# mmetcalf14/qml-cutensornet

Measured on AMD Instinct MI355X. Metric: Gram kernel entries/sec @ 60 qubits x 6 layers, higher is better.
Workload: dtype f64 (complex128)

## Files before the change

### __graft_entry__.py

```python
from __future__ import annotations

import os
import shutil
import subprocess
import sys

ROOT = os.path.dirname(os.path.abspath(__file__))
PKG = os.path.join(ROOT, "qml-cutensornet_amd")
if ROOT not in sys.path:
    sys.path.insert(0, ROOT)


def _run(cmd):
    print("+", " ".join(cmd), file=sys.stderr, flush=True)
    subprocess.run(cmd, check=True)


def _stale(out, deps):
    return not os.path.exists(out) or os.path.getmtime(out) < max(os.path.getmtime(f) for f in deps)


def build_variant(name, defines) -> str:
    build()
    hipcc = shutil.which("hipcc") or "/opt/rocm/bin/hipcc"
    csrc, lab = os.path.join(PKG, "csrc"), os.path.join(ROOT, "lab")
    obj, out = os.path.join(lab, f"qkgram_{name}.o"), os.path.join(lab, f"libqkgram_{name}.so")
    srcs = [os.path.join(csrc, f) for f in ("qkgram.hip", "qk_fused.h", "qk_ring.h", "qk_device.h", "qk_host.h", "qk_devmem.h", "qk_plan.h")] + [os.path.join(lab, "qk_quad.h")]
    if _stale(out, srcs):
        _run([hipcc, "--offload-arch=gfx950", "-O3", "-std=c++17", "-fPIC", "-DQKF_EXPERIMENT", "-I", lab] + [f"-D{d}" for d in defines] + ["-c", "-o", obj, srcs[0]])
        _run([hipcc, "--offload-arch=gfx950", "-shared", "-fPIC", "-o", out, obj] + [os.path.join(csrc, f) for f in ("qk_build.o", "qk_comm.o", "qk_local.o", "qk_planner.o")] + ["-ldl", "-lpthread"])
    return out


def build() -> None:
    hipcc = shutil.which("hipcc") or "/opt/rocm/bin/hipcc"
    csrc = os.path.join(PKG, "csrc")
    lab = os.path.join(ROOT, "lab")
    inc = os.path.join(ROOT, "include", "qkgram.h")
    common = [os.path.join(csrc, h) for h in ("qk_host.h", "qk_devmem.h", "qk_plan.h", "qk_device.h")] + [inc]
    deps = {
        "qkgram.hip": common + [os.path.join(csrc, h) for h in ("qk_ring.h", "qk_fused.h")],
        "qk_build.hip": common + [os.path.join(csrc, "qk_build_kernels.h")],
        "qk_comm.hip": common,
        "qk_local.hip": common + [os.path.join(csrc, "qk_ring.h")],
    }
    gxx = shutil.which("g++") or "g++"
    psrc, pobj = os.path.join(csrc, "qk_planner.cpp"), os.path.join(csrc, "qk_planner.o")
    if _stale(pobj, [psrc, os.path.join(csrc, "qk_plan.h"), inc]):
        _run([gxx, "-O3", "-std=c++17", "-fPIC", "-pthread", "-fopenmp-simd", "-c", "-o", pobj, psrc])
    targets = [(os.path.join(PKG, "libqkgram.so"), "", [], [])]
    if os.path.exists(os.path.join(lab, "qk_lab.hip")):
        targets.append((os.path.join(lab, "libqklab.so"), ".lab", ["-DQK_LAB", "-I", csrc, "-I", lab], [os.path.join(lab, "qk_lab.hip")]))
    for out, tag, flags, extra in targets:
        objs = []
        for src in [os.path.join(csrc, f) for f in deps] + extra:
            obj = os.path.splitext(src)[0] + tag + ".o"
            d = deps.get(os.path.basename(src), deps["qkgram.hip"] + [os.path.join(lab, "qk_lab.h")])
            if _stale(obj, [src] + d):
                _run([hipcc, "--offload-arch=gfx950", "-O3", "-std=c++17", "-fPIC"] + flags + ["-c", "-o", obj, src])
            objs.append(obj)
        if _stale(out, objs + [pobj]):
            _run([hipcc, "--offload-arch=gfx950", "-shared", "-fPIC", "-o", out] + objs + [pobj, "-ldl", "-lpthread"])
    bsrc = os.path.join(csrc, "qk_builder.cpp")
    bout = os.path.join(PKG, "libqkbuilder.so")
    if not os.path.exists(bout) or os.path.getmtime(bout) < os.path.getmtime(bsrc):
        _run([shutil.which("g++") or "g++", "-O3", "-std=c++17", "-shared", "-fPIC", "-o", bout, bsrc, "-ldl"])
    omk = os.path.join(ROOT, "oracle", "Makefile")
    if os.path.exists(omk):
        _run(["make", "-s", "-C", os.path.join(ROOT, "oracle")])
    import qml_cutensornet_amd
    from qml_cutensornet_amd import engine

    engine.lib()


def smoke() -> None:
    import numpy as np

    build()
    import qml_cutensornet_amd as Q
    from qml_cutensornet_amd import engine
    from oracle import restatement as R

    with engine.context(0) as ctx:
        ctx.selftest()
        for n, reps, gamma, d, npts, want in ((10, 2, 1.0, 2, 6, "wave"), (14, 4, 1.0, 3, 5, "fused")):
# ... 20 lines not shown
```

### lab/qk_quad.h

```cpp
#pragma once

__device__ __forceinline__ int qkq_qinv(const int d) {
  static constexpr int T[17] = {0, 1048576, 524288, 349526, 262144, 209716, 174763, 149797, 131072, 116509, 104858, 95326, 87382, 80660, 74899, 69906, 65536};
  return T[d];
}

struct QkqUnit {
  bool mine, a1, b1;
  int ta, tb, p;
};

template <bool A1, bool B1, typename XPtr>
__device__ __forceinline__ void qkq_p1(QkfTile (&T)[2][2], v2d (&fr)[4], v2d (&fs)[4], const bool primed, QkfStream cur, XPtr xp, unsigned x0, unsigned x1, const int nks,
                                       const QkfStream n0, const unsigned n1off) {
  v4d P[2][2][3];
  v2d fx[4], fy[4];
  if (!primed) qkf_load4(fr, cur);
  if (B1) {
#pragma unroll
    for (int i = 0; i < 4; ++i) fs[i] = qkf_ldg(cur.base + i * cur.step, cur.off + TILE);
  }
#pragma unroll
  for (int i = 0; i < 4; ++i) {
    fx[i] = qkf_ldx(xp + i * QKF_XSTEP, x0);
// ... 224 lines not shown
    if (cut) {
      if (un.b1) un.tb += sub, un.b1 = false;
      else if (un.a1) un.ta += sub, un.a1 = false;
      else un.mine = un.mine && sub == 0;
    }
    return un;
  };
  auto b_stream = [&](const QkfSite& s, const int s0, const QkqUnit& un) __attribute__((always_inline)) {
    return QkfStream{s.Bk + un.p * s.b2, (unsigned)((q * s.pd) * s.b2 + (s0 + un.tb) * TILE + j), 4 * s.pd * s.b2};
  };
  auto a_stream = [&](const QkfSite& s, const QkqUnit& un) __attribute__((always_inline)) {
    return QkfStream{s.Ak + un.p * s.a2, (unsigned)(((un.ta * TILE + q) * s.pd) * s.a2 + j), 4 * s.pd * s.a2};
  };
  const int xcc = qk_xcc_id();
  if (tid == 0) qk_tail_start(g);
  for (;;) {
    if (tid == 0) *slot = qk_pull(g, xcc);
    __syncthreads();
    const long long p = *slot;
    __syncthreads();
    if (p < 0) break;
    const int xi = g.pairs[2 * p], yj = g.pairs[2 * p + 1];
    qkf_step_table<XCAP, NT>(g, xi, yj, rec, m_off, tid, [](const int pmt, const int nt) { return pmt * ((nt + 1) / 2) <= NW; });
    const int ek = g.edge_k, k_hi = ns - ek;
    const bool edges = ek > 0;
    if (!edges)
      for (int e = tid; e < TILE * TILE; e += NT) XL[e] = (v2d){e == 0 ? 1.0 : 0.0, 0.0};
    __syncthreads();
    bool xg = false;
    int cur = 0, xb = 0;
    if (edges) {
      const v4i r0 = rec[3 * ek];
      const int a_e = rfl(r0.x), b_e = rfl(r0.z);
      if (a_e * b_e <= XCAP) qkf_edge_prefix<NW>(g, xi, yj, a_e, b_e, XL, wave, q, j);
      else qkf_edge_prefix<NW>(g, xi, yj, a_e, b_e, G0, wave, q, j), xg = true;
      __syncthreads();
    }
    v2d fr[4], fs[4];
    bool primed = false;
    QkfSite sn = site(ek);
    for (int k = ek; k < k_hi;) {
      const QkfSite sc = sn;
      k = sc.next;
      if (k < k_hi) sn = site(k);
      const int a = sc.a, a2 = sc.a2, b = sc.b, nt = sc.nt, W = sc.W;
      const bool small = sc.small;
      v2d* const Gc = G0 + (long long)cur * g.x_plane;
      v2d* const Gn = G0 + (long long)(cur ^ 1) * g.x_plane;
      if (small && xg) {
        for (int e = tid; e < a * b; e += NT) XL[e] = Gc[e];
        __syncthreads();
        xg = false, xb = 0;
      } else if (!small && !xg) {
        for (int e = tid; e < a * b; e += NT) Gc[e] = XL[xb + e];
        __syncthreads();
        xg = true;
      }
      const int n_out = sc.b2 * a2;
      const bool pingpong = small && a * b + n_out <= XCAP;
      const int ob = !small ? 0 : pingpong ? (xb == 0 ? XCAP - n_out : 0) : 0;
      if (pingpong)
        for (int e = tid; e < n_out; e += NT) XL[ob + e] = (v2d){0.0, 0.0};
      for (int s0 = 0; s0 < nt; s0 += W) {
        const int w = min(W, nt - s0);
        const Pieces pc = pieces_of(sc, w);
        const int quads = pc.L;
        if (!small) {
          for (int e = tid; e < w * TILE * a2; e += NT) XL[e] = (v2d){0.0, 0.0};
// ... 49 lines not shown
              constexpr bool A1_ = decltype(a1_)::value, B1_ = decltype(b1_)::value;
              if (kmax == 4) qkq_p2<true, A1_, B1_>(T, fr, fs, as, a1off, ps, sc.nn, 4, xo, q, j, nxt);
              else qkq_p2<false, A1_, B1_>(T, fr, fs, as, a1off, ps, sc.nn, kmax, xo, q, j, nxt);
            };
            if (un.a1) {
              if (un.b1) p2(std::true_type{}, std::true_type{});
              else p2(std::true_type{}, std::false_type{});
            } else {
              if (un.b1) p2(std::false_type{}, std::true_type{});
              else p2(std::false_type{}, std::false_type{});
            }
            primed = np1;
          } else {
            between();
          }
        }
        qk_lds_barrier();
        if (!small && nt > W) {
          for (int tn = 0; tn < sc.nn; ++tn)
            for (int e = tid; e < w * QKF_XBLOCK; e += NT) Gn[(long long)tn * (sc.b2 * TILE) + s0 * QKF_XBLOCK + e] = XL[tn * w * QKF_XBLOCK + e];
          __syncthreads();
        }
      }
      if (!small) {
        if (nt > W) cur ^= 1;
        else xg = false, xb = 0;
      } else {
        xb = ob;
      }
    }
    if (edges) {
      const v4i r0 = rec[3 * (k_hi - 1)];
      const int a_e = rfl(r0.y), b_e = rfl(r0.w);
      if (xg) qkf_edge_suffix<NW>(g, xi, yj, a_e, b_e, (const v2d*)(G0 + (long long)cur * g.x_plane), zacc, wave, q, j);
      else qkf_edge_suffix<NW>(g, xi, yj, a_e, b_e, (const lds_v2d*)(XL + xb), zacc, wave, q, j);
      __syncthreads();
    }
    if (tid == 0) {
      v2d zz = {0.0, 0.0};
      if (edges)
        for (int w_ = 0; w_ < NW; ++w_) zz.x += zacc[2 * w_], zz.y += zacc[2 * w_ + 1];
      else zz = xg ? G0[(long long)cur * g.x_plane] : (v2d)XL[xb];
      g.values[p] = zz.x * zz.x + zz.y * zz.y;
      if (g.z) {
        g.z[2 * p] = zz.x;
        g.z[2 * p + 1] = zz.y;
      }
    }
    __syncthreads();
  }
  if (tid == 0) qk_tail_exit(g);
}
```

### qml-cutensornet_amd/csrc/qk_fused.h

```cpp
#pragma once
#include "qk_device.h"
#include "qk_plan.h"

#define QKF_PRIO_LO() __builtin_amdgcn_s_setprio(0)
#define QKF_PRIO_HI() __builtin_amdgcn_s_setprio(2)
typedef double v2d __attribute__((ext_vector_type(2)));
typedef __attribute__((address_space(3))) v2d lds_v2d;
static constexpr int QKF_XSTEP = 4 * TILE;
static constexpr int QKF_XBLOCK = TILE * TILE;


#ifndef QKF_LDS3M
#define QKF_LDS3M 0
#endif
#ifndef QKF_P2_PROBE
#define QKF_P2_PROBE 0
#endif
#ifndef QKF_ABL
#define QKF_ABL 0
#endif
#define QKF_STEP_BARRIER()                            \
  do {                                                \
    if (QKF_ABL & 4) asm volatile("s_waitcnt lgkmcnt(0)" ::: "memory"); \
    else qk_lds_barrier();                            \
// ... 189 lines not shown
      for (int r = 0; r < 4; ++r) {
        __hip_atomic_fetch_add(d + r * 2 * QKF_XSTEP, re[r], __ATOMIC_RELAXED, __HIP_MEMORY_SCOPE_WORKGROUP);
        __hip_atomic_fetch_add(d + r * 2 * QKF_XSTEP + 1, im[r], __ATOMIC_RELAXED, __HIP_MEMORY_SCOPE_WORKGROUP);
      }
    }
    d += 2 * ps;
  }
}

template <int S>
__device__ __forceinline__ void qkf_rotate(QkfTile (&T)[S], const int L) {
  if constexpr (S >= 2) {
    if (L == 2) {
      const QkfTile t = T[S - 2];
      T[S - 2] = T[S - 1], T[S - 1] = t;
    }
  }
  if constexpr (S >= 3) {
    if (L == 3) {
      const QkfTile t = T[S - 3];
      T[S - 3] = T[S - 2], T[S - 2] = T[S - 1], T[S - 1] = t;
    }
  }
  if constexpr (S >= 4) {
    if (L >= 4) {
      const QkfTile t0 = T[0];
#pragma unroll
      for (int e = 0; e + 1 < S; ++e) T[e] = T[e + 1];
      T[S - 1] = t0;
    }
  }
}

__device__ __forceinline__ void qkf_edge_tile(QkfTile& t, const v2d* __restrict__ Ay, const int ldy, const v2d* __restrict__ Ax, const int ldx, const int ks4) {
  v4d p1 = {0, 0, 0, 0}, p2 = {0, 0, 0, 0}, p3 = {0, 0, 0, 0};
  v2d fy[4], fx[4];
#pragma unroll
  for (int i = 0; i < 4; ++i) fy[i] = Ay[(long)(4 * i) * ldy], fx[i] = Ax[(long)(4 * i) * ldx];
  for (int s0 = 0; s0 < ks4; s0 += 4) {
    const bool more = s0 + 4 < ks4;
#pragma unroll
    for (int i = 0; i < 4; ++i) {
      qkf_kstep<true>(p1, p2, p3, fy[i].x, fy[i].y, fx[i].x, fx[i].y);
      if (more) fy[i] = Ay[(long)(4 * (s0 + 4 + i)) * ldy], fx[i] = Ax[(long)(4 * (s0 + 4 + i)) * ldx];
    }
  }
  t.re = p1 + p2, t.im = p3 - p1 + p2;
}

template <int NW, typename XOut>
__device__ __forceinline__ void qkf_edge_prefix(const SweepArgs& g, const int xi, const int yj, const int a, const int b, XOut xo, const int wave, const int q, const int j) {
  const v2d* const Lx = reinterpret_cast<const v2d*>(g.xedge) + g.xedge_offs[2 * (long long)xi];
  const v2d* const Ly = reinterpret_cast<const v2d*>(g.yedge) + g.yedge_offs[2 * (long long)yj];
  const int mt = a / TILE, nt = b / TILE, ks4 = (1 << g.edge_k) >> 2;
  for (int t = wave; t < mt * nt; t += NW) {
    const int tb = t / mt, ta = t - tb * mt;
    QkfTile T;
    qkf_edge_tile(T, Ly + (long)q * b + tb * TILE + j, b, Lx + (long)q * a + ta * TILE + j, a, ks4);
#pragma unroll
    for (int r = 0; r < 4; ++r) xo[ta * (b * TILE) + (tb * TILE + q + 4 * r) * TILE + j] = (v2d){T.re[r], T.im[r]};
  }
}

template <int NW, typename XIn>
__device__ __forceinline__ void qkf_edge_suffix(const SweepArgs& g, const int xi, const int yj, const int a, const int b, XIn xin, __attribute__((address_space(3))) double* zacc, const int wave,
                                                const int q, const int j) {
  const v2d* const Rx = reinterpret_cast<const v2d*>(g.xedge) + g.xedge_offs[2 * (long long)xi + 1];
  const v2d* const Ry = reinterpret_cast<const v2d*>(g.yedge) + g.yedge_offs[2 * (long long)yj + 1];
  const int mt = a / TILE, nt = b / TILE, ks4 = (1 << g.edge_k) >> 2;
  double zr = 0, zi = 0;
  for (int t = wave; t < mt * nt; t += NW) {
    const int tb = t / mt, ta = t - tb * mt;
    QkfTile T;
    qkf_edge_tile(T, Ry + (long)q * b + tb * TILE + j, b, Rx + (long)q * a + ta * TILE + j, a, ks4);
#pragma unroll
    for (int r = 0; r < 4; ++r) {
      const v2d x = xin[ta * (b * TILE) + (tb * TILE + q + 4 * r) * TILE + j];
      zr += x.x * T.re[r] - x.y * T.im[r], zi += x.x * T.im[r] + x.y * T.re[r];
    }
  }
#pragma unroll
  for (int o = 32; o > 0; o >>= 1) zr += __shfl_xor(zr, o), zi += __shfl_xor(zi, o);
  if ((q | j) == 0) zacc[2 * wave] = zr, zacc[2 * wave + 1] = zi;
}

struct QkfSite {
  int a, a2, b, b2, at, nks, mt, nt, nn, W, inv, inv2, pd, ps, next;
  bool small;
  const v2d *Ak, *Bk;
};
typedef int v4i __attribute__((ext_vector_type(4)));
typedef __attribute__((address_space(3))) v4i lds_v4i;

template <int XCAP, int NT, bool ITEM_RECIPS = false, typename OneRound>
__device__ __forceinline__ void qkf_step_table(const SweepArgs& g, const int xi, const int yj, lds_v4i* const rec, long long* const m_off, const int tid, const OneRound one_round) {
  const int ns = g.n_sites, n1 = ns + 1;
  const int32_t* const xd = g.xdims + (long long)xi * n1;
  const int32_t* const yd = g.ydims + (long long)yj * n1;
  const int32_t* const xt = g.xtrue + (long long)xi * n1;
  const int32_t* const yt = g.ytrue + (long long)yj * n1;
  const v2d* const xdata = reinterpret_cast<const v2d*>(g.xdata);
  const v2d* const ydata = reinterpret_cast<const v2d*>(g.ydata);
  auto is_small = [&](const int a, const int a2, const int b, const int b2, const int pd) __attribute__((always_inline)) {
    return a * b <= XCAP && a2 * b2 <= XCAP && (one_round(pd * (a / TILE), b2 / TILE) || a * b + a2 * b2 <= XCAP);
  };
  auto put = [&](const int e, const int a, const int a2, const int b, const int b2, const int ps, const int next, const bool small, const v2d* const A, const v2d* const B)
                 __attribute__((always_inline)) {
    const int mt = a / TILE, nt = b2 / TILE;
    const int W = small ? nt : max(1, min(nt, XCAP / (TILE * a2)));
    rec[3 * e] = (v4i){a, a2, b, b2};
    rec[3 * e + 1] = (v4i){xt[e], (yt[e] + 3) >> 2, W, small ? 1 : 0};
// ... 20 lines not shown
    const bool sm = is_small(a, a2, b, b2, 4);
    const long long work_m = 4ll * a * b2 * (b + a2), work_p = 2ll * a * bm * (b + am) + 2ll * am * b2 * (bm + a2);
    const bool merged = (sm || (!is_small(a, am, b, bm, 2) && !is_small(am, a2, bm, b2, 2))) && work_m <= work_p;
    plain(e + 1, e + 2);
    if (merged)
      put(e, a, a2, b, b2, 2, e + 2, sm, reinterpret_cast<const v2d*>(g.xmg) + (g.xmg_offs[(long long)xi * g.merge_steps + t] >> 1),
          reinterpret_cast<const v2d*>(g.ymg) + (g.ymg_offs[(long long)yj * g.merge_steps + t] >> 1));
    else plain(e, e + 1);
  }
}

#ifdef QKF_PROF
#define QKF_PROF_DECL() \
  unsigned long long pf[8] = {0, 0, 0, 0, 0, 0, 0, 0}, pt = __builtin_amdgcn_s_memtime(); \
  const unsigned long long pt0 = pt
#define QKF_STAMP(i)                                              \
  do {                                                            \
    const unsigned long long now_ = __builtin_amdgcn_s_memtime(); \
    pf[i] += now_ - pt;                                           \
    pt = now_;                                                    \
  } while (0)
#define QKF_PROF_FLUSH()                                             \
  do {                                                               \
    if (lane == 0) {                                                 \
      pf[7] = __builtin_amdgcn_s_memtime() - pt0;                    \
      for (int i_ = 0; i_ < 8; ++i_) atomicAdd(g.prof + i_, pf[i_]); \
    }                                                                \
  } while (0)
#else
#define QKF_PROF_DECL()
#define QKF_STAMP(i)
#define QKF_PROF_FLUSH()
#endif

template <int NW, int S, int XCAP, int WPS, bool DET = false>
__global__ __launch_bounds__(64 * NW, WPS) void qk_sweep_fused_kernel(const SweepArgs g) {
  constexpr int NT = 64 * NW;
  extern __shared__ __attribute__((aligned(16))) double lds_raw[];
  lds_v2d* const XL = (lds_v2d*)lds_raw;
  long long* const slot = reinterpret_cast<long long*>(lds_raw + 2 * XCAP);
  const v2d* const xdata = reinterpret_cast<const v2d*>(g.xdata);
  const v2d* const ydata = reinterpret_cast<const v2d*>(g.ydata);
  v2d* const G0 = reinterpret_cast<v2d*>(g.scratch) + (long long)blockIdx.x * 2 * g.x_plane;
  const int tid = threadIdx.x, lane = tid & 63;
  const int wave = __builtin_amdgcn_readfirstlane(tid >> 6);
  const int j = lane & 15, q = lane >> 4;
  const int ns = g.n_sites;
  __attribute__((address_space(3))) double* const zacc = (__attribute__((address_space(3))) double*)(slot + 2);
  lds_v4i* const rec = (lds_v4i*)(slot + 2 + 32);
  long long* const m_off = reinterpret_cast<long long*>(slot + 2 + 32) + 6 * (long long)ns;
  lds_int* const tbroken = (lds_int*)(m_off + 2 * (long long)ns);
  lds_int* const turn0 = tbroken + 2;
  auto rfl = [&](const int v) __attribute__((always_inline)) { return __builtin_amdgcn_readfirstlane(v); };
  auto ldl = [&](const long long* p_) __attribute__((always_inline)) {
    const long long v = *p_;
    const unsigned lo = __builtin_amdgcn_readfirstlane((unsigned)v);
    const unsigned hi = __builtin_amdgcn_readfirstlane((unsigned)((unsigned long long)v >> 32));
    return (long long)(((unsigned long long)hi << 32) | lo);
  };
  auto site = [&](const int k) __attribute__((always_inline)) {
    const v4i r0 = rec[3 * k], r1 = rec[3 * k + 1], r2 = rec[3 * k + 2];
    QkfSite s;
    s.a = rfl(r0.x), s.a2 = rfl(r0.y), s.b = rfl(r0.z), s.b2 = rfl(r0.w);
    s.at = rfl(r1.x), s.nks = rfl(r1.y), s.W = rfl(r1.z), s.small = rfl(r1.w) != 0;
    s.inv = rfl(r2.x), s.inv2 = rfl(r2.w);
    s.ps = rfl(r2.y), s.pd = 1 << s.ps, s.next = rfl(r2.z);
// ... 12 lines not shown
  auto a_stream = [&](const QkfSite& s, const int w, const int it) __attribute__((always_inline)) {
    const QkUnit un = item_of(s, w, it);
    return QkfStream{s.Ak + un.p * s.a2, (unsigned)(((un.ta * TILE + q) * s.pd) * s.a2 + j), 4 * s.pd * s.a2, min(4, (s.at - un.ta * TILE + 3) >> 2)};
  };
  QKF_PROF_DECL();
  const int xcc = qk_xcc_id();
  int gang_round = 0;
  if (tid == 0) qk_tail_start(g);
  for (;;) {
    if (tid == 0) {
      const long long pp_ = qk_pull(g, xcc);
      qk_gang_sync(g, xcc, pp_ >= 0, gang_round);
      *slot = pp_;
    }
    __syncthreads();
    const long long p = *slot;
    __syncthreads();
    if (p < 0) break;
    const int xi = g.pairs[2 * p], yj = g.pairs[2 * p + 1];
    qkf_step_table<XCAP, NT, true>(g, xi, yj, rec, m_off, tid, [](const int pmt, const int nt) { return pmt * nt <= NW * S; });
    const int ek = g.edge_k, k_hi = ns - ek;
    const bool edges = ek > 0;
    if (!edges)
      for (int e = tid; e < TILE * TILE; e += NT) XL[e] = (v2d){e == 0 ? 1.0 : 0.0, 0.0};
    if constexpr (DET)
      for (int e = tid; e < 2 * g.turn_ints + 2; e += NT) tbroken[e] = 0;
    int tsel = 0;
    __syncthreads();
    bool xg = false;
    int cur = 0, xb = 0;
    if (edges) {
      const v4i r0 = rec[3 * ek];
      const int a_e = rfl(r0.x), b_e = rfl(r0.z);
      if (a_e * b_e <= XCAP) qkf_edge_prefix<NW>(g, xi, yj, a_e, b_e, XL, wave, q, j);
      else qkf_edge_prefix<NW>(g, xi, yj, a_e, b_e, G0, wave, q, j), xg = true;
      __syncthreads();
    }
    QKF_STAMP(0);
    QkfTile T[S];
    v2d fr[4];
    bool primed = false;
    QkfSite sn = site(ek);
    for (int k = ek; k < k_hi;) {
      const QkfSite sc = sn;
      k = sc.next;
      if (k < k_hi) sn = site(k);
      const int a = sc.a, a2 = sc.a2, b = sc.b, mt = sc.mt, nt = sc.nt, W = sc.W;
      const bool small = sc.small;
      v2d* const Gc = G0 + (long long)cur * g.x_plane;
      v2d* const Gn = G0 + (long long)(cur ^ 1) * g.x_plane;
      if (small && xg) {
        for (int e = tid; e < a * b; e += NT) XL[e] = Gc[e];
        __syncthreads();
        xg = false, xb = 0;
      } else if (!small && !xg) {
        for (int e = tid; e < a * b; e += NT) Gc[e] = XL[xb + e];
        __syncthreads();
        xg = true;
      }
      const int n_out = sc.b2 * a2;
      const bool pingpong = small && a * b + n_out <= XCAP;
      const int ob = !small ? 0 : pingpong ? (xb == 0 ? XCAP - n_out : 0) : 0;
      if (pingpong && !DET)
        for (int e = tid; e < n_out; e += NT) XL[ob + e] = (v2d){0.0, 0.0};
      QKF_STAMP(1);
      for (int s0 = 0; s0 < nt; s0 += W) {
        const int w = min(W, nt - s0), items = sc.pd * mt * w;
        lds_int* const tcur = turn0 + tsel * g.turn_ints;
// ... 44 lines not shown
            const int kmax = min(4, (sc.at - ta * TILE + 3) >> 2);
            const bool more = s + 1 < S && it + NW < items;
            const int wn = min(sn.W, sn.nt);
            const bool chain = !more && last_round && k < k_hi && wave < sn.pd * sn.mt * wn;
            const QkfStream nxt = more ? a_stream(sc, w, it + NW) : chain ? b_stream(sn, 0, wn, wave) : a_stream(sc, w, it);
            const int tix = sc.pd * ta + un.p;
            const QkfTurn turn{tcur + tbl * sc.nn, tix, tbroken, g.err};
            if (kmax == 4) qkf_p2_item<true, DET>(T[S - 1], fr, primed, a_stream(sc, w, it), w * QKF_XBLOCK, sc.nn, 4, XL + ob + tbl * QKF_XBLOCK, q, j, nxt, turn);
            else qkf_p2_item<false, DET>(T[S - 1], fr, primed, a_stream(sc, w, it), w * QKF_XBLOCK, sc.nn, kmax, XL + ob + tbl * QKF_XBLOCK, q, j, nxt, turn);
            primed = more || chain;
          }
          QKF_STAMP(4);
        }
        QKF_STEP_BARRIER();
        tsel ^= 1;
        QKF_STAMP(5);
        if (!small && nt > W) {
          for (int tn = 0; tn < sc.nn; ++tn)
            for (int e = tid; e < w * QKF_XBLOCK; e += NT) Gn[(long long)tn * (sc.b2 * TILE) + s0 * QKF_XBLOCK + e] = XL[tn * w * QKF_XBLOCK + e];
          __syncthreads();
          QKF_STAMP(1);
        }
      }
      if (!small) {
        if (nt > W) cur ^= 1;
        else xg = false, xb = 0;
      } else {
        xb = ob;
      }
    }
    if (edges) {
      const v4i r0 = rec[3 * (k_hi - 1)];
      const int a_e = rfl(r0.y), b_e = rfl(r0.w);
      if (xg) qkf_edge_suffix<NW>(g, xi, yj, a_e, b_e, (const v2d*)(G0 + (long long)cur * g.x_plane), zacc, wave, q, j);
      else qkf_edge_suffix<NW>(g, xi, yj, a_e, b_e, (const lds_v2d*)(XL + xb), zacc, wave, q, j);
      __syncthreads();
    }
    if (tid == 0) {
      v2d zz = {0.0, 0.0};
      if (edges)
        for (int w_ = 0; w_ < NW; ++w_) zz.x += zacc[2 * w_], zz.y += zacc[2 * w_ + 1];
      else zz = xg ? G0[(long long)cur * g.x_plane] : (v2d)XL[xb];
      g.values[p] = zz.x * zz.x + zz.y * zz.y;
      if (g.z) {
        g.z[2 * p] = zz.x;
        g.z[2 * p + 1] = zz.y;
      }
    }
    __syncthreads();
  }
  if (tid == 0) qk_tail_exit(g);
  QKF_PROF_FLUSH();
}

template <bool HAS1, typename XPtr>
__device__ __forceinline__ void qkf_p1_dual(QkfTile& t0, QkfTile& t1, v2d (&fr)[4], v2d (&fs)[4], const bool primed, QkfStream cur, XPtr xp, unsigned xoff, const int nks,
                                            const QkfStream nxt) {
  v4d p1 = {0, 0, 0, 0}, p2 = {0, 0, 0, 0}, p3 = {0, 0, 0, 0}, r1 = {0, 0, 0, 0}, r2 = {0, 0, 0, 0}, r3 = {0, 0, 0, 0};
  v2d fx[4];
  if (!primed) qkf_load4(fr, cur);
  if (HAS1) {
#pragma unroll
    for (int i = 0; i < 4; ++i) fs[i] = qkf_ldg(cur.base + i * cur.step, cur.off + TILE);
  }
#pragma unroll
  for (int i = 0; i < 4; ++i) fx[i] = qkf_ldx(xp + i * QKF_XSTEP, xoff);
  const int ng = (nks + 3) >> 2, last = nks - 4 * (ng - 1);
  QKF_PRIO_LO();
// ... 245 lines not shown
    s.Ak = xdata + ldl(m_off + 2 * k);
    s.Bk = ydata + ldl(m_off + 2 * k + 1);
    return s;
  };
  auto pair_of = [&](const QkfSite& s, const int v) __attribute__((always_inline)) { return qk_unit_decode_ordered(v, s.ps, s.mt, s.inv); };
  auto b_stream = [&](const QkfSite& s, const int s0, const int v, const int half) __attribute__((always_inline)) {
    const QkUnit un = pair_of(s, v);
    return QkfStream{s.Bk + un.p * s.b2, (unsigned)((q * s.pd) * s.b2 + (s0 + 2 * un.tc + half) * TILE + j), 4 * s.pd * s.b2};
  };
  struct Unit {
    bool mine, has1;
    int v, half;
  };
  auto unit_of = [&](const QkfSite& s, const int w, const int units, const int r0) __attribute__((always_inline)) {
    Unit un;
    const int left = units - r0;
    const bool halves = 2 * left <= NW;
    un.half = (halves && wave >= left) ? 1 : 0;
    un.v = r0 + wave - (un.half ? left : 0);
    const int tp = pair_of(s, un.v).tc;
    const bool second = 2 * tp + 1 < w;
    un.mine = un.v < units && (un.half == 0 || second);
    un.has1 = !halves && second;
    return un;
  };
  auto a_stream = [&](const QkfSite& s, const int v) __attribute__((always_inline)) {
    const QkUnit un = pair_of(s, v);
    return QkfStream{s.Ak + un.p * s.a2, (unsigned)(((un.ta * TILE + q) * s.pd) * s.a2 + j), 4 * s.pd * s.a2};
  };
  QKF_PROF_DECL();
  const int xcc = qk_xcc_id();
  int gang_round = 0;
  if (tid == 0) qk_tail_start(g);
  for (;;) {
    if (tid == 0) {
      const long long pp_ = qk_pull(g, xcc);
      qk_gang_sync(g, xcc, pp_ >= 0, gang_round);
      *slot = pp_;
    }
    __syncthreads();
    const long long p = *slot;
    __syncthreads();
    if (p < 0) break;
    const int xi = g.pairs[2 * p], yj = g.pairs[2 * p + 1];
    qkf_step_table<XCAP, NT>(g, xi, yj, rec, m_off, tid, [](const int pmt, const int nt) { return pmt * ((nt + 1) / 2) <= NW; });
    const int ek = g.edge_k, k_hi = ns - ek;
    const bool edges = ek > 0;
    if (!edges)
      for (int e = tid; e < TILE * TILE; e += NT) XL[e] = (v2d){e == 0 ? 1.0 : 0.0, 0.0};
    if constexpr (DET)
      for (int e = tid; e < 2 * g.turn_ints + 2; e += NT) tbroken[e] = 0;
    int tsel = 0;
    __syncthreads();
    bool xg = false;
    int cur = 0, xb = 0;
    if (edges) {
      const v4i r0 = rec[3 * ek];
      const int a_e = rfl(r0.x), b_e = rfl(r0.z);
      if (a_e * b_e <= XCAP) qkf_edge_prefix<NW>(g, xi, yj, a_e, b_e, XL, wave, q, j);
      else qkf_edge_prefix<NW>(g, xi, yj, a_e, b_e, G0, wave, q, j), xg = true;
      __syncthreads();
    }
    QKF_STAMP(0);
    QkfTile T0, T1;
    v2d fr[4], fs[4];
    bool primed = false;
    QkfSite sn = site(ek);
    for (int k = ek; k < k_hi;) {
      const QkfSite sc = sn;
      k = sc.next;
      if (k < k_hi) sn = site(k);
      const int a = sc.a, a2 = sc.a2, b = sc.b, mt = sc.mt, nt = sc.nt, W = sc.W;
      const bool small = sc.small;
      v2d* const Gc = G0 + (long long)cur * g.x_plane;
      v2d* const Gn = G0 + (long long)(cur ^ 1) * g.x_plane;
      if (small && xg) {
        for (int e = tid; e < a * b; e += NT) XL[e] = Gc[e];
        __syncthreads();
        xg = false, xb = 0;
      } else if (!small && !xg) {
        for (int e = tid; e < a * b; e += NT) Gc[e] = XL[xb + e];
        __syncthreads();
        xg = true;
      }
      const int n_out = sc.b2 * a2;
      const bool pingpong = small && a * b + n_out <= XCAP;
      const int ob = !small ? 0 : pingpong ? (xb == 0 ? XCAP - n_out : 0) : 0;
      if (pingpong && !DET)
        for (int e = tid; e < n_out; e += NT) XL[ob + e] = (v2d){0.0, 0.0};
      QKF_STAMP(1);
      for (int s0 = 0; s0 < nt; s0 += W) {
        const int w = min(W, nt - s0), units = sc.pd * mt * ((w + 1) >> 1);
        lds_int* const tcur = turn0 + tsel * g.turn_ints;
// ... 45 lines not shown
              const Unit nu = unit_of(sn, w2, sn.pd * sn.mt * ((w2 + 1) >> 1), 0);
              if (nu.mine) nxt = b_stream(sn, 0, nu.v, nu.half), np1 = true;
            }
            const unsigned nd1 = 0;
            lds_v2d* const xo = XL + ob + (2 * tp + un.half) * QKF_XBLOCK;
            const QkfTurn tp_turn{tcur + (2 * tp + un.half) * sc.nn, sc.pd * ta + pr.p, tbroken, g.err};
            if (has1) {
              if (kmax == 4) qkf_p2_dual<true, true, DET>(T0, T1, fr, fs, a_stream(sc, v), w * QKF_XBLOCK, sc.nn, 4, xo, q, j, nxt, np1, nd1, tp_turn);
              else qkf_p2_dual<false, true, DET>(T0, T1, fr, fs, a_stream(sc, v), w * QKF_XBLOCK, sc.nn, kmax, xo, q, j, nxt, np1, nd1, tp_turn);
            } else {
              if (kmax == 4) qkf_p2_dual<true, false, DET>(T0, T1, fr, fs, a_stream(sc, v), w * QKF_XBLOCK, sc.nn, 4, xo, q, j, nxt, np1, nd1, tp_turn);
              else qkf_p2_dual<false, false, DET>(T0, T1, fr, fs, a_stream(sc, v), w * QKF_XBLOCK, sc.nn, kmax, xo, q, j, nxt, np1, nd1, tp_turn);
            }
            primed = np1;
          }
          QKF_STAMP(4);
        }
        QKF_STEP_BARRIER();
        tsel ^= 1;
        QKF_STAMP(5);
        if (!small && nt > W) {
          for (int tn = 0; tn < sc.nn; ++tn)
            for (int e = tid; e < w * QKF_XBLOCK; e += NT) Gn[(long long)tn * (sc.b2 * TILE) + s0 * QKF_XBLOCK + e] = XL[tn * w * QKF_XBLOCK + e];
          __syncthreads();
        }
      }
      if (!small) {
        if (nt > W) cur ^= 1;
        else xg = false, xb = 0;
      } else {
        xb = ob;
      }
    }
    if (edges) {
      const v4i r0 = rec[3 * (k_hi - 1)];
      const int a_e = rfl(r0.y), b_e = rfl(r0.w);
      if (xg) qkf_edge_suffix<NW>(g, xi, yj, a_e, b_e, (const v2d*)(G0 + (long long)cur * g.x_plane), zacc, wave, q, j);
      else qkf_edge_suffix<NW>(g, xi, yj, a_e, b_e, (const lds_v2d*)(XL + xb), zacc, wave, q, j);
      __syncthreads();
    }
    if (tid == 0) {
      v2d zz = {0.0, 0.0};
      if (edges)
        for (int w_ = 0; w_ < NW; ++w_) zz.x += zacc[2 * w_], zz.y += zacc[2 * w_ + 1];
      else zz = xg ? G0[(long long)cur * g.x_plane] : (v2d)XL[xb];
      g.values[p] = zz.x * zz.x + zz.y * zz.y;
      if (g.z) {
        g.z[2 * p] = zz.x;
        g.z[2 * p + 1] = zz.y;
      }
    }
    __syncthreads();
    QKF_STAMP(6);
  }
  if (tid == 0) qk_tail_exit(g);
  QKF_PROF_FLUSH();
}

template <typename T>
__global__ void qk_interleave_kernel(const T* __restrict__ src, T* __restrict__ dst, const int32_t* __restrict__ dims, const int64_t* __restrict__ offs,
                                     const int n_sites, const long long n_tensors) {
  typedef T v2 __attribute__((ext_vector_type(2)));
  for (long long t = blockIdx.x; t < n_tensors; t += gridDim.x) {
    const long long s = t / n_sites;
    const int k = (int)(t - s * n_sites);
    const long long plane = (long long)dims[s * (n_sites + 1) + k] * 2 * dims[s * (n_sites + 1) + k + 1];
    const T* re = src + offs[t];
    const T* im = re + plane;
    v2* d = reinterpret_cast<v2*>(dst + offs[t]);
    for (long long e = threadIdx.x; e < plane; e += blockDim.x) d[e] = (v2){re[e], im[e]};
  }
}

template <int N>
__device__ __forceinline__ void qkw_wait_vmcnt() {
  static_assert(N >= 0 && N < 64, "vmcnt is a 6-bit field");
  asm volatile("s_waitcnt vmcnt(%0)" ::"n"(N) : "memory");
}

template <int NG, typename SRC>
__global__ __launch_bounds__(64, 2) void qk_sweep_wave2_kernel(const SweepArgs g) {
  constexpr bool F32 = sizeof(SRC) == 4;
  static_assert(!F32 || NG > 0, "complex64 images go through the LDS ring");
  constexpr int ES = F32 ? 8 : 16;
  constexpr int GROUP = F32 ? 128 : 256;
// ... 195 lines not shown
```

### qml-cutensornet_amd/csrc/qk_plan.h

```cpp
#pragma once
#include "../../include/qkgram.h"

#include <algorithm>
#include <cstdint>
#include <cstdio>
#include <vector>

int qk_fail(int code, const char* fmt, ...) __attribute__((format(printf, 2, 3)));

#ifndef QKF_XCAP_ONE_V
#define QKF_XCAP_ONE_V 8192
#endif
#ifndef QKF_XCAP_TWO_V
#define QKF_XCAP_TWO_V 4608
#endif
#ifndef QKF_TWO_WGS
#define QKF_TWO_WGS 2
#endif
static constexpr int QKF_XCAP_ONE = QKF_XCAP_ONE_V, QKF_XCAP_TWO = QKF_XCAP_TWO_V;
static constexpr int QK_TILE = 16;
static inline int qk_pad16(int x) { return (x + QK_TILE - 1) / QK_TILE * QK_TILE; }
static constexpr int GMAX = 4;

#if defined(__HIPCC__)
#define QK_HD __host__ __device__
#else
#define QK_HD
#endif
struct QkUnit {
  int ta, tc, p;
};
QK_HD static inline int qk_unit_cols(const int w, const bool dual) { return dual ? (w + 1) >> 1 : w; }
QK_HD static inline int qk_recip20(const int d) { return ((1 << 20) + d - 1) / d; }
QK_HD static inline int qk_recip15(const int d) { return ((1 << 15) + d - 1) / d; }
QK_HD static inline int qk_unit_recips(const int nt, const int W, const bool dual) {
  const int wl = nt - (nt - 1) / W * W;
  return qk_recip15(qk_unit_cols(W, dual)) | (qk_recip15(qk_unit_cols(wl, dual)) << 16);
}
QK_HD static inline int qk_unit_recip_of(const int recips, const bool full_strip) { return full_strip ? (recips & 0xffff) : (int)((unsigned)recips >> 16); }
QK_HD static inline QkUnit qk_unit_decode(const int v, const int mt, const int wc, const int inv_mt, const int inv_wc) {
  const int c = (v * inv_mt) >> 20, p = (c * inv_wc) >> 15;
  return QkUnit{v - c * mt, c - p * wc, p};
}
QK_HD static inline QkUnit qk_unit_decode_ordered(const int v, const int ps, const int mt, const int inv_mt) {
  const int u = v >> ps, tc = (u * inv_mt) >> 20;
  return QkUnit{u - tc * mt, tc, v & ((1 << ps) - 1)};
}

struct qk_ctx;

struct qk_plan {
  int n_sites = 0, nx = 0, ny = 0;
  bool symmetric = false;
  bool quad = false;
  int world = 1, rank = 0;
  int64_t total_pairs = 0, max_per_rank = 0;
  std::vector<int32_t> pairs;
  std::vector<int32_t> groups;
  int group = 1;
  qk_stats stats{};
  qk_stats second{};
  int64_t n_first = 0;
  int nq = 1;
  int64_t qstart[17] = {0};
  int edge_k = 0;
  bool second_wave2 = false;
  double fit_two = 1.0;
  double fit_narrow = 1.0;
  double tile_reuse_bytes = 0;
  double plan_ms = 0;
  int plan_threads = 1;
  qk_ctx* up_ctx = nullptr;
  int32_t* d_pairs = nullptr;
  int32_t* d_groups = nullptr;
};

struct QkSweepPolicy {
  int variant = 20;
  int wgs_per_cu = 2;
// ... 114 lines not shown
```

Measured before the change: 712,000.

## Rewrite edge prefix/suffix with pipelined MFMA groups and prefetch next pair

Replaces the edge tile contraction with a unit-based version that keeps one or two groups of k-step loads in flight, uses byte-offset addressing and scalarised base offsets, and can optionally compute two column tiles per unit. In the gang fused kernel, a dedicated puller thread fetches the next work pair during the suffix phase and the step table for the next pair is built before looping, which removes a barrier per pair. The aim is to hide global-load latency in the edge contractions and the scheduler round-trip. It adds register pressure and more complex control flow, and it changes the synchronisation ordering.

```diff
diff --git a/__graft_entry__.py b/__graft_entry__.py
--- a/__graft_entry__.py
+++ b/__graft_entry__.py
@@ -52,6 +52,9 @@
     if os.path.exists(os.path.join(lab, "qk_lab.hip")):
         targets.append((os.path.join(lab, "libqklab.so"), ".lab", ["-DQK_LAB", "-I", csrc, "-I", lab], [os.path.join(lab, "qk_lab.hip")]))
     for out, tag, flags, extra in targets:
+        every = {f for src in deps for f in [os.path.join(csrc, src)] + deps[src]} | set(extra) | {psrc, os.path.join(lab, "qk_lab.h"), os.path.join(lab, "qk_quad.h")}
+        if not _stale(out, [f for f in every if os.path.exists(f)]):
+            continue
         objs = []
         for src in [os.path.join(csrc, f) for f in deps] + extra:
             obj = os.path.splitext(src)[0] + tag + ".o"
diff --git a/lab/qk_quad.h b/lab/qk_quad.h
--- a/lab/qk_quad.h
+++ b/lab/qk_quad.h
@@ -280,8 +280,8 @@
     if (edges) {
       const v4i r0 = rec[3 * ek];
       const int a_e = rfl(r0.x), b_e = rfl(r0.z);
-      if (a_e * b_e <= XCAP) qkf_edge_prefix<NW>(g, xi, yj, a_e, b_e, XL, wave, q, j);
-      else qkf_edge_prefix<NW>(g, xi, yj, a_e, b_e, G0, wave, q, j), xg = true;
+      xg = a_e * b_e > XCAP;
+      qkf_edge_prefix<NW, QKF_EDGE_PAIRS(WPS), QKF_EDGE_SETS(WPS)>(g, xi, yj, a_e, b_e, XL, G0, xg, wave, q, j);
       __syncthreads();
     }
     v2d fr[4], fs[4];
@@ -397,8 +397,7 @@
     if (edges) {
       const v4i r0 = rec[3 * (k_hi - 1)];
       const int a_e = rfl(r0.y), b_e = rfl(r0.w);
-      if (xg) qkf_edge_suffix<NW>(g, xi, yj, a_e, b_e, (const v2d*)(G0 + (long long)cur * g.x_plane), zacc, wave, q, j);
-      else qkf_edge_suffix<NW>(g, xi, yj, a_e, b_e, (const lds_v2d*)(XL + xb), zacc, wave, q, j);
+      qkf_edge_suffix<NW, QKF_EDGE_PAIRS(WPS), QKF_EDGE_SETS(WPS)>(g, xi, yj, a_e, b_e, (const lds_v2d*)(XL + xb), (const v2d*)(G0 + (long long)cur * g.x_plane), xg, zacc, wave, q, j);
       __syncthreads();
     }
     if (tid == 0) {
diff --git a/qml-cutensornet_amd/csrc/qk_fused.h b/qml-cutensornet_amd/csrc/qk_fused.h
--- a/qml-cutensornet_amd/csrc/qk_fused.h
+++ b/qml-cutensornet_amd/csrc/qk_fused.h
@@ -245,51 +245,151 @@
   }
 }
 
-__device__ __forceinline__ void qkf_edge_tile(QkfTile& t, const v2d* __restrict__ Ay, const int ldy, const v2d* __restrict__ Ax, const int ldx, const int ks4) {
-  v4d p1 = {0, 0, 0, 0}, p2 = {0, 0, 0, 0}, p3 = {0, 0, 0, 0};
-  v2d fy[4], fx[4];
-#pragma unroll
-  for (int i = 0; i < 4; ++i) fy[i] = Ay[(long)(4 * i) * ldy], fx[i] = Ax[(long)(4 * i) * ldx];
-  for (int s0 = 0; s0 < ks4; s0 += 4) {
-    const bool more = s0 + 4 < ks4;
-#pragma unroll
-    for (int i = 0; i < 4; ++i) {
-      qkf_kstep<true>(p1, p2, p3, fy[i].x, fy[i].y, fx[i].x, fx[i].y);
-      if (more) fy[i] = Ay[(long)(4 * (s0 + 4 + i)) * ldy], fx[i] = Ax[(long)(4 * (s0 + 4 + i)) * ldx];
-    }
-  }
-  t.re = p1 + p2, t.im = p3 - p1 + p2;
-}
-
-template <int NW, typename XOut>
-__device__ __forceinline__ void qkf_edge_prefix(const SweepArgs& g, const int xi, const int yj, const int a, const int b, XOut xo, const int wave, const int q, const int j) {
-  const v2d* const Lx = reinterpret_cast<const v2d*>(g.xedge) + g.xedge_offs[2 * (long long)xi];
-  const v2d* const Ly = reinterpret_cast<const v2d*>(g.yedge) + g.yedge_offs[2 * (long long)yj];
-  const int mt = a / TILE, nt = b / TILE, ks4 = (1 << g.edge_k) >> 2;
-  for (int t = wave; t < mt * nt; t += NW) {
-    const int tb = t / mt, ta = t - tb * mt;
-    QkfTile T;
-    qkf_edge_tile(T, Ly + (long)q * b + tb * TILE + j, b, Lx + (long)q * a + ta * TILE + j, a, ks4);
-#pragma unroll
-    for (int r = 0; r < 4; ++r) xo[ta * (b * TILE) + (tb * TILE + q + 4 * r) * TILE + j] = (v2d){T.re[r], T.im[r]};
-  }
-}
-
-template <int NW, typename XIn>
-__device__ __forceinline__ void qkf_edge_suffix(const SweepArgs& g, const int xi, const int yj, const int a, const int b, XIn xin, __attribute__((address_space(3))) double* zacc, const int wave,
+#ifdef QKF_EDGE_PAIRS_V
+#define QKF_EDGE_PAIRS(WPS) (QKF_EDGE_PAIRS_V != 0)
+#else
+#define QKF_EDGE_PAIRS(WPS) false
+#endif
+#ifdef QKF_EDGE_SETS_V
+#define QKF_EDGE_SETS(WPS) (QKF_EDGE_SETS_V)
+#else
+#define QKF_EDGE_SETS(WPS) ((WPS) <= 3 ? 2 : 1)
+#endif
+__device__ __forceinline__ v2d qkf_lde(const v2d* __restrict__ base, const unsigned boff, const int col = 0) {
+  return reinterpret_cast<const v2d*>(reinterpret_cast<const char*>(base) + (size_t)boff)[col];
+}
+template <bool HAS1, bool MORE>
+__device__ __forceinline__ void qkf_edge_group(v4d (&acc)[6], v2d (&fy)[4], v2d (&fz)[4], v2d (&fx)[4], const v2d* const* const by, const v2d* const* const bx, const unsigned boy,
+                                               const unsigned box) {
+#pragma unroll
+  for (int i = 0; i < 4; ++i) {
+    const double sb = QKF_DIF(fx[i].x, fx[i].y);
+    acc[0] = __builtin_amdgcn_mfma_f64_16x16x4f64(fy[i].x, fx[i].x, acc[0], 0, 0, 0);
+    acc[1] = __builtin_amdgcn_mfma_f64_16x16x4f64(fy[i].y, fx[i].y, acc[1], 0, 0, 0);
+    acc[2] = __builtin_amdgcn_mfma_f64_16x16x4f64(QKF_SUM(fy[i].x, fy[i].y), sb, acc[2], 0, 0, 0);
+    if (HAS1) {
+      acc[3] = __builtin_amdgcn_mfma_f64_16x16x4f64(fz[i].x, fx[i].x, acc[3], 0, 0, 0);
+      acc[4] = __builtin_amdgcn_mfma_f64_16x16x4f64(fz[i].y, fx[i].y, acc[4], 0, 0, 0);
+      acc[5] = __builtin_amdgcn_mfma_f64_16x16x4f64(QKF_SUM(fz[i].x, fz[i].y), sb, acc[5], 0, 0, 0);
+    }
+    if (MORE) {
+      fy[i] = qkf_lde(by[i], boy);
+      if (HAS1) fz[i] = qkf_lde(by[i], boy, TILE);
+      fx[i] = qkf_lde(bx[i], box);
+    }
+    __builtin_amdgcn_sched_barrier(0);
+  }
+}
+template <bool HAS1, int SETS>
+__device__ __forceinline__ void qkf_edge_unit(QkfTile& t0, QkfTile& t1, const v2d* __restrict__ Ay, const unsigned oy, const int ldy, const v2d* __restrict__ Ax, const unsigned ox, const int ldx,
+                                              const int ng) {
+  static_assert(SETS == 1 || SETS == 2, "one or two groups of k-steps in flight");
+  v4d acc[6];
+#pragma unroll
+  for (int e = 0; e < 6; ++e) acc[e] = (v4d){0, 0, 0, 0};
+  v2d fy[SETS][4], fz[SETS][4], fx[SETS][4];
+  const v2d *by[4 * SETS], *bx[4 * SETS];
+#pragma unroll
+  for (int i = 0; i < 4 * SETS; ++i) by[i] = Ay + 4 * i * ldy, bx[i] = Ax + 4 * i * ldx;
+  unsigned boy = oy * 16u, box = ox * 16u;
+  const unsigned sy = (unsigned)(SETS * TILE * ldy) * 16u, sx = (unsigned)(SETS * TILE * ldx) * 16u;
+  const bool two = SETS == 2 && ng > 1;
+#pragma unroll
+  for (int s = 0; s < SETS; ++s) {
+    if (s == 0 || two) {
+#pragma unroll
+      for (int i = 0; i < 4; ++i) {
+        fy[s][i] = qkf_lde(by[4 * s + i], boy);
+        if (HAS1) fz[s][i] = qkf_lde(by[4 * s + i], boy, TILE);
+        fx[s][i] = qkf_lde(bx[4 * s + i], box);
+      }
+    }
+  }
+  QKF_PRIO_LO();
+#pragma unroll 1
+  for (int g = SETS; g < ng; g += SETS) {
+    boy += sy, box += sx;
+#pragma unroll
+    for (int s = 0; s < SETS; ++s) qkf_edge_group<HAS1, true>(acc, fy[s], fz[s], fx[s], by + 4 * s, bx + 4 * s, boy, box);
+  }
+  qkf_edge_group<HAS1, false>(acc, fy[0], fz[0], fx[0], by, bx, boy, box);
+  if constexpr (SETS == 2) {
+    if (two) qkf_edge_group<HAS1, false>(acc, fy[1], fz[1], fx[1], by + 4, bx + 4, boy, box);
+  }
+  QKF_PRIO_HI();
+  t0.re = acc[0] + acc[1], t0.im = acc[2] - acc[0] + acc[1];
+  if (HAS1) t1.re = acc[3] + acc[4], t1.im = acc[5] - acc[3] + acc[4];
+}
+__device__ __forceinline__ long long qkf_uniform(const long long v) {
+  const unsigned lo = __builtin_amdgcn_readfirstlane((unsigned)v);
+  const unsigned hi = __builtin_amdgcn_readfirstlane((unsigned)((unsigned long long)v >> 32));
+  return (long long)(((unsigned long long)hi << 32) | lo);
+}
+
+template <int NW, bool PAIRS>
+__device__ __forceinline__ QkEdgeUnit qkf_edge_unit_of(const int u, const int mt, const int nt, const int inv) {
+  if constexpr (PAIRS) return qk_edge_unit(u, mt, nt, NW, inv);
+  const int tb = (u * inv) >> 20;
+  return QkEdgeUnit{u - tb * mt, tb, false, true};
+}
+template <int NW, bool PAIRS, int SETS>
+__device__ __forceinline__ void qkf_edge_prefix(const SweepArgs& g, const int xi, const int yj, const int a, const int b, lds_v2d* const xl, v2d* const xg, const bool to_global, const int wave,
                                                 const int q, const int j) {
-  const v2d* const Rx = reinterpret_cast<const v2d*>(g.xedge) + g.xedge_offs[2 * (long long)xi + 1];
-  const v2d* const Ry = reinterpret_cast<const v2d*>(g.yedge) + g.yedge_offs[2 * (long long)yj + 1];
-  const int mt = a / TILE, nt = b / TILE, ks4 = (1 << g.edge_k) >> 2;
+  const v2d* const Lx = reinterpret_cast<const v2d*>(g.xedge) + qkf_uniform(g.xedge_offs[2 * (long long)xi]);
+  const v2d* const Ly = reinterpret_cast<const v2d*>(g.yedge) + qkf_uniform(g.yedge_offs[2 * (long long)yj]);
+  const int mt = a / TILE, nt = b / TILE, ng = (1 << g.edge_k) >> 4, inv = qk_recip20(mt), units = PAIRS ? qk_edge_units(mt, nt, NW) : mt * nt;
+  for (int u = wave; u < units; u += NW) {
+    const QkEdgeUnit un = qkf_edge_unit_of<NW, PAIRS>(u, mt, nt, inv);
+    if (!un.mine) continue;
+    QkfTile T0, T1;
+    const unsigned oy = (unsigned)(q * b + un.tb0 * TILE + j), ox = (unsigned)(q * a + un.ta * TILE + j);
+    if (un.has1) qkf_edge_unit<true, 1>(T0, T1, Ly, oy, b, Lx, ox, a, ng);
+    else qkf_edge_unit<false, SETS>(T0, T1, Ly, oy, b, Lx, ox, a, ng);
+    const int at = un.ta * (b * TILE) + (un.tb0 * TILE + q) * TILE + j;
+    if (to_global) {
+#pragma unroll
+      for (int r = 0; r < 4; ++r) xg[at + r * QKF_XSTEP] = (v2d){T0.re[r], T0.im[r]};
+      if (un.has1) {
+#pragma unroll
+        for (int r = 0; r < 4; ++r) xg[at + QKF_XBLOCK + r * QKF_XSTEP] = (v2d){T1.re[r], T1.im[r]};
+      }
+    } else {
+#pragma unroll
+      for (int r = 0; r < 4; ++r) xl[at + r * QKF_XSTEP] = (v2d){T0.re[r], T0.im[r]};
+      if (un.has1) {
+#pragma unroll
+        for (int r = 0; r < 4; ++r) xl[at + QKF_XBLOCK + r * QKF_XSTEP] = (v2d){T1.re[r], T1.im[r]};
+      }
+    }
+  }
+}
+
+template <int NW, bool PAIRS, int SETS>
+__device__ __forceinline__ void qkf_edge_suffix(const SweepArgs& g, const int xi, const int yj, const int a, const int b, const lds_v2d* const xl, const v2d* const xg, const bool from_global,
+                                                __attribute__((address_space(3))) double* zacc, const int wave, const int q, const int j) {
+  const v2d* const Rx = reinterpret_cast<const v2d*>(g.xedge) + qkf_uniform(g.xedge_offs[2 * (long long)xi + 1]);
+  const v2d* const Ry = reinterpret_cast<const v2d*>(g.yedge) + qkf_uniform(g.yedge_offs[2 * (long long)yj + 1]);
+  const int mt = a / TILE, nt = b / TILE, ng = (1 << g.edge_k) >> 4, inv = qk_recip20(mt), units = PAIRS ? qk_edge_units(mt, nt, NW) : mt * nt;
   double zr = 0, zi = 0;
-  for (int t = wave; t < mt * nt; t += NW) {
-    const int tb = t / mt, ta = t - tb * mt;
-    QkfTile T;
-    qkf_edge_tile(T, Ry + (long)q * b + tb * TILE + j, b, Rx + (long)q * a + ta * TILE + j, a, ks4);
+  for (int u = wave; u < units; u += NW) {
+    const QkEdgeUnit un = qkf_edge_unit_of<NW, PAIRS>(u, mt, nt, inv);
+    if (!un.mine) continue;
+    QkfTile T0, T1;
+    const unsigned oy = (unsigned)(q * b + un.tb0 * TILE + j), ox = (unsigned)(q * a + un.ta * TILE + j);
+    if (un.has1) qkf_edge_unit<true, 1>(T0, T1, Ry, oy, b, Rx, ox, a, ng);
+    else qkf_edge_unit<false, SETS>(T0, T1, Ry, oy, b, Rx, ox, a, ng);
+    const int at = un.ta * (b * TILE) + (un.tb0 * TILE + q) * TILE + j;
 #pragma unroll
     for (int r = 0; r < 4; ++r) {
-      const v2d x = xin[ta * (b * TILE) + (tb * TILE + q + 4 * r) * TILE + j];
-      zr += x.x * T.re[r] - x.y * T.im[r], zi += x.x * T.im[r] + x.y * T.re[r];
+      const v2d x = from_global ? xg[at + r * QKF_XSTEP] : (v2d)xl[at + r * QKF_XSTEP];
+      zr += x.x * T0.re[r] - x.y * T0.im[r], zi += x.x * T0.im[r] + x.y * T0.re[r];
+    }
+    if (un.has1) {
+#pragma unroll
+      for (int r = 0; r < 4; ++r) {
+        const v2d x = from_global ? xg[at + QKF_XBLOCK + r * QKF_XSTEP] : (v2d)xl[at + QKF_XBLOCK + r * QKF_XSTEP];
+        zr += x.x * T1.re[r] - x.y * T1.im[r], zi += x.x * T1.im[r] + x.y * T1.re[r];
+      }
     }
   }
 #pragma unroll
@@ -376,6 +476,13 @@
 #define QKF_STAMP(i)
 #define QKF_PROF_FLUSH()
 #endif
+
+#define QKF_PULLER(NT) ((NT) - 64)
+__device__ __forceinline__ void qkf_pull_next(const SweepArgs& g, const int xcc, int& gang_round, long long* const word) {
+  const long long pp = qk_pull(g, xcc);
+  qk_gang_sync(g, xcc, pp >= 0, gang_round);
+  *word = pp;
+}
 
 template <int NW, int S, int XCAP, int WPS, bool DET = false>
 __global__ __launch_bounds__(64 * NW, WPS) void qk_sweep_fused_kernel(const SweepArgs g) {
@@ -454,8 +561,8 @@
     if (edges) {
       const v4i r0 = rec[3 * ek];
       const int a_e = rfl(r0.x), b_e = rfl(r0.z);
-      if (a_e * b_e <= XCAP) qkf_edge_prefix<NW>(g, xi, yj, a_e, b_e, XL, wave, q, j);
-      else qkf_edge_prefix<NW>(g, xi, yj, a_e, b_e, G0, wave, q, j), xg = true;
+      xg = a_e * b_e > XCAP;
+      qkf_edge_prefix<NW, QKF_EDGE_PAIRS(WPS), QKF_EDGE_SETS(WPS)>(g, xi, yj, a_e, b_e, XL, G0, xg, wave, q, j);
       __syncthreads();
     }
     QKF_STAMP(0);
@@ -566,8 +673,7 @@
     if (edges) {
       const v4i r0 = rec[3 * (k_hi - 1)];
       const int a_e = rfl(r0.y), b_e = rfl(r0.w);
-      if (xg) qkf_edge_suffix<NW>(g, xi, yj, a_e, b_e, (const v2d*)(G0 + (long long)cur * g.x_plane), zacc, wave, q, j);
-      else qkf_edge_suffix<NW>(g, xi, yj, a_e, b_e, (const lds_v2d*)(XL + xb), zacc, wave, q, j);
+      qkf_edge_suffix<NW, QKF_EDGE_PAIRS(WPS), QKF_EDGE_SETS(WPS)>(g, xi, yj, a_e, b_e, (const lds_v2d*)(XL + xb), (const v2d*)(G0 + (long long)cur * g.x_plane), xg, zacc, wave, q, j);
       __syncthreads();
     }
     if (tid == 0) {
@@ -879,18 +985,18 @@
   const int xcc = qk_xcc_id();
   int gang_round = 0;
   if (tid == 0) qk_tail_start(g);
-  for (;;) {
-    if (tid == 0) {
-      const long long pp_ = qk_pull(g, xcc);
-      qk_gang_sync(g, xcc, pp_ >= 0, gang_round);
-      *slot = pp_;
-    }
-    __syncthreads();
-    const long long p = *slot;
-    __syncthreads();
-    if (p < 0) break;
+  if (tid == QKF_PULLER(NT)) qkf_pull_next(g, xcc, gang_round, slot);
+  __syncthreads();
+  long long p = slot[0];
+  int psel = 0;
+  auto table_of = [&](const long long pp) __attribute__((always_inline)) {
+    if (pp < 0) return;
+    const int xi_ = g.pairs[2 * pp], yj_ = g.pairs[2 * pp + 1];
+    qkf_step_table<XCAP, NT>(g, xi_, yj_, rec, m_off, tid, [](const int pmt, const int nt) { return pmt * ((nt + 1) / 2) <= NW; });
+  };
+  table_of(p);
+  while (p >= 0) {
     const int xi = g.pairs[2 * p], yj = g.pairs[2 * p + 1];
-    qkf_step_table<XCAP, NT>(g, xi, yj, rec, m_off, tid, [](const int pmt, const int nt) { return pmt * ((nt + 1) / 2) <= NW; });
     const int ek = g.edge_k, k_hi = ns - ek;
     const bool edges = ek > 0;
     if (!edges)
@@ -904,8 +1010,8 @@
     if (edges) {
       const v4i r0 = rec[3 * ek];
       const int a_e = rfl(r0.x), b_e = rfl(r0.z);
-      if (a_e * b_e <= XCAP) qkf_edge_prefix<NW>(g, xi, yj, a_e, b_e, XL, wave, q, j);
-      else qkf_edge_prefix<NW>(g, xi, yj, a_e, b_e, G0, wave, q, j), xg = true;
+      xg = a_e * b_e > XCAP;
+      qkf_edge_prefix<NW, QKF_EDGE_PAIRS(WPS), QKF_EDGE_SETS(WPS)>(g, xi, yj, a_e, b_e, XL, G0, xg, wave, q, j);
       __syncthreads();
     }
     QKF_STAMP(0);
@@ -1017,13 +1123,14 @@
         xb = ob;
       }
     }
+    if (tid == QKF_PULLER(NT)) qkf_pull_next(g, xcc, gang_round, slot + (psel ^ 1));
     if (edges) {
       const v4i r0 = rec[3 * (k_hi - 1)];
       const int a_e = rfl(r0.y), b_e = rfl(r0.w);
-      if (xg) qkf_edge_suffix<NW>(g, xi, yj, a_e, b_e, (const v2d*)(G0 + (long long)cur * g.x_plane), zacc, wave, q, j);
-      else qkf_edge_suffix<NW>(g, xi, yj, a_e, b_e, (const lds_v2d*)(XL + xb), zacc, wave, q, j);
-      __syncthreads();
-    }
+      qkf_edge_suffix<NW, QKF_EDGE_PAIRS(WPS), QKF_EDGE_SETS(WPS)>(g, xi, yj, a_e, b_e, (const lds_v2d*)(XL + xb), (const v2d*)(G0 + (long long)cur * g.x_plane), xg, zacc, wave, q, j);
+    }
+    __syncthreads();
+    const long long pn = slot[psel ^ 1];
     if (tid == 0) {
       v2d zz = {0.0, 0.0};
       if (edges)
@@ -1035,7 +1142,9 @@
         g.z[2 * p + 1] = zz.y;
       }
     }
-    __syncthreads();
+    table_of(pn);
+    if (!edges) __syncthreads();
+    p = pn, psel ^= 1;
     QKF_STAMP(6);
   }
   if (tid == 0) qk_tail_exit(g);
diff --git a/qml-cutensornet_amd/csrc/qk_plan.h b/qml-cutensornet_amd/csrc/qk_plan.h
--- a/qml-cutensornet_amd/csrc/qk_plan.h
+++ b/qml-cutensornet_amd/csrc/qk_plan.h
@@ -45,6 +45,22 @@
 QK_HD static inline QkUnit qk_unit_decode_ordered(const int v, const int ps, const int mt, const int inv_mt) {
   const int u = v >> ps, tc = (u * inv_mt) >> 20;
   return QkUnit{u - tc * mt, tc, v & ((1 << ps) - 1)};
+}
+
+struct QkEdgeUnit {
+  int ta, tb0;
+  bool has1, mine;
+};
+QK_HD static inline int qk_edge_units(const int mt, const int nt, const int NW) {
+  const int pairs = mt * ((nt + 1) >> 1), r0 = (pairs - 1) / NW * NW, left = pairs - r0;
+  return 2 * left <= NW ? r0 + 2 * left : pairs;
+}
+QK_HD static inline QkEdgeUnit qk_edge_unit(const int u, const int mt, const int nt, const int NW, const int inv_mt) {
+  const int pairs = mt * ((nt + 1) >> 1), r0 = (pairs - 1) / NW * NW, left = pairs - r0;
+  const bool halves = 2 * left <= NW, single = halves && u >= r0, half = halves && u >= r0 + left;
+  const int v = u - (half ? left : 0), tp = (v * inv_mt) >> 20;
+  const bool second = 2 * tp + 1 < nt;
+  return QkEdgeUnit{v - tp * mt, 2 * tp + (half ? 1 : 0), !single && second, u < (halves ? r0 + 2 * left : pairs) && (!half || second)};
 }
 
 struct qk_ctx;
```

Measured after the change: 733,900 (median of 6 runs). +3.1%, better.
